# chenkovsky/aha

Measured on AMD Instinct MI355X. Metric: input GB/s scanned + M-hits/s, 100k-pattern AC over 1 GiB UTF-8 corpus, higher is better.
Workload: dtype u8

## Files before the change

### aha_amd/csrc/engine.cpp

```cpp
#include "handle.hpp"

#include <chrono>

namespace ahai {

constexpr size_t kLdsPerCU = 160 * 1024;
constexpr uint64_t kV2MaxRegionBytes = 48ull << 30;

bool skip_eligible(const aha_ac *ac) {
  const UnitImage &u = ac->unit;
  if (!u.ok || u.base_bits != 22 || u.unit_key || u.mark_bloom.empty()) return false;
  const char *eng = getenv("AHA_ENGINE");
  if (eng && strcmp(eng, "skip") != 0) return false;
  const char *hb = getenv("AHA_UNIT_HEADER_BESIDE");
  if (hb ? atoi(hb) != 0 : (!eng && (uint64_t)u.n_nfr * 5 >= u.n_states)) return false;
  const char *sk = getenv("AHA_SKIP");
  if (sk) return atoi(sk) != 0;
  return eng != nullptr;
}

bool pair_eligible(const aha_ac *ac) {
  const UnitImage &u = ac->unit;
  if (!u.ok || u.base_bits != 22 || u.unit_key || u.pair_tab.empty() || u.mark_bloom.empty() || u.deep_ends_max > kPairMaxDeepEnds ||
      ac->aut.max_key_len > 255)
// ... 297 lines not shown
  z[kSlabUsed] = direct ? 0 : n_slabs * 4;
  z[kEvCnt] = n_chunks * 4;
  z[kDocEvRank] = n_docs1 * 4;
  z[kEvBase] = n_chunks * 8;
  z[kBlkA] = z[kBlkB] = n_blk * 8;
  z[kCursor] = kCursorBytes;
  z[kEvAux] = z[kSortedAux] = chars ? ev_cap * 4 : 0;
  z[kLeadCnt] = z[kChunkDoc0] = (chars || pair) ? n_chunks * 4 : 0;
  z[kDocLeadRank] = chars ? n_docs1 * 4 : 0;
  z[kLeadBase] = chars ? n_chunks * 8 : 0;
  z[kEvRegions] = (unit && ac->unit_fused) ? 0 : n_reg * 8;
  z[kText] = 0;
  z[kChunkHits] = direct ? n_chunks * 4 : 0;
  z[kHitBase] = direct ? n_chunks * 8 : 0;
  z[kDocHitRank] = unit ? n_docs1 * 4 : 0;
  z[kEvGroups] = unit ? n_reg * 12 : 0;
  z[kEngineA] = filt ? ((N + 63) / 64 + 2) * 8 : (skip ? skip_bitmap_bytes(N) : (pair ? n_chunks * 4 : 0));
  z[kEngineB] = filt ? n_chunks * filter_chunk_rec_bytes() : (pair ? pair_cand_bytes(cand_cap) : 0);
  z[kEngineC] = pair ? pair_walk_bytes(cand_cap) : 0;
  z[kKeyVisits] = 0;
  return 0;
}

constexpr int32_t kNoRegions = 5;
static int32_t launch_v2(aha_ac *ac, Scratch *sc, MatchArgs &M1, const V2Plan &P, V2Args &M, bool prof, hipStream_t s) {
  const uint64_t N = M1.n_bytes;
  const bool counting = M1.count_only != 0, direct = P.direct, filt = P.filt, pair = P.pair, unit = P.unit, skip = P.skip;
  M = V2Args{};
  M.doc_off = M1.doc_off;
  M.n_docs = M1.n_docs;
  M.n_bytes = N;
  M.S = (uint32_t)P.S;
  M.n_chunks = P.n_chunks;
  M.lds_slots = ac->v2_lds_slots;
  M.chars = M1.chars;
  M.sep = M1.sep;
  memcpy(M.sep_block, M1.sep_block, sizeof(M.sep_block));
  M.out = M1.out;
  M.cap = M1.cap;
  M.doc_hit_off = M1.doc_hit_off;
  M.unit_bb = ac->unit.base_bits;
  M.direct = direct ? 1 : 0;
  M.dense_hits = P.dense ? 1 : 0;
  M.ev_stride = (uint32_t)P.stride;
  M.ev_cap = P.ev_cap;
  int32_t rc;
  for (int i = 0; i < kV2Count; i++) {
    if (!P.sizes[i]) continue;
    if ((rc = v2_reserve(sc, (V2Slot)i, P.sizes[i]))) return ((i == kEvRegions || i == kEvGroups) && P.mode != kSlabs) ? kNoRegions : rc;
  }
  if (M1.fold && !filt && (rc = stage_folded(ac, sc, M1, s))) return rc;
  const bool fold_loads = filt && M1.fold;
  auto at = [sc](V2Slot slot) { return sc->v2buf[slot].p; };
  M.text = M1.text;
  M.ev = (uint4 *)at(kEv);
  M.sorted_ev = (uint4 *)at(kSortedEv);
  M.sorted_cnt = (uint32_t *)at(kSortedCnt);
  M.slab_used = (uint32_t *)at(kSlabUsed);
  M.ev_cnt = (uint32_t *)at(kEvCnt);
  M.doc_ev_rank = (uint32_t *)at(kDocEvRank);
  M.ev_base = (uint64_t *)at(kEvBase);
  M.blk_a = (uint64_t *)at(kBlkA);
  M.blk_b = (uint64_t *)at(kBlkB);
  if (sc->cursor_buf != at(kCursor)) {
    sc->cursor_buf = at(kCursor);
    sc->cursor_dirty = true;
  }
  M.ev_aux = (uint32_t *)at(kEvAux);
  M.sorted_aux = (uint32_t *)at(kSortedAux);
  M.lead_cnt = (uint32_t *)at(kLeadCnt);
  M.chunk_doc0 = (uint32_t *)at(kChunkDoc0);
  M.doc_lead_rank = (uint32_t *)at(kDocLeadRank);
  M.lead_base = (uint64_t *)at(kLeadBase);
  M.evd = (uint2 *)at(kEvRegions);
  M.evg = (uint32_t *)at(kEvGroups);
  M.doc_hit_rank = (uint32_t *)at(kDocHitRank);
  M.chunk_hits = (uint32_t *)at(kChunkHits);
  M.hit_base = (uint64_t *)at(kHitBase);
  if ((rc = ensure_h_v2(ac, sc))) return rc;
  M.publish = (direct && M.doc_hit_off && sc->h_v2_dev) ? sc->h_v2_dev : nullptr;
  static const bool always_clear = getenv("AHA_CURSOR_MEMSET") != nullptr;
  if (sc->cursor_dirty || always_clear) {
    HIPCHK(ac, hipMemsetAsync(at(kCursor), 0, kCursorBytes, s));
    sc->cursor_phase = 0;
  }
  M.cursor = (unsigned long long *)at(kCursor) + 16 * sc->cursor_phase;
  M.totals = (uint64_t *)M.cursor + 2;
  M.clear_next = M.publish ? (unsigned long long *)at(kCursor) + 16 * (sc->cursor_phase ^ 1u) : nullptr;
  sc->cursor_dirty = true;

  if (M1.check_docs) launch_check_docs(M.doc_off, M.n_docs, N, nullptr, M.cursor + 1, s);
  if (M1.kc_visits) HIPCHK(ac, hipMemsetAsync(M1.kc_visits, 0, (size_t)ac->aut.n_keys * 8, s));
  if (prof) HIPCHK(ac, hipEventRecord(sc->ev[0], s));
  const uint64_t n_tiles = (M.n_chunks + kV2Threads - 1) / kV2Threads;
  DevAut post = ac->dev;
  if (pair) {
    post.end_info = ac->d_unit_end_info;
    post.compact = 1;
    pair_launch(ac->pdev, ac->udev, post, M, at(kEngineA), at(kEngineB), at(kEngineC), P.cand_cap, ac->v2_grid,
                prof ? (void *)sc->ev[2] : nullptr, s);
  } else if (unit) {
    post.end_info = ac->d_unit_end_info;
    post.compact = 1;
    if (skip) {
      skip_launch_mark(ac->sdev, M, at(kEngineA), ac->v2_grid, s);
      if (prof) HIPCHK(ac, hipEventRecord(sc->ev[2], s));
      skip_launch_traverse(ac->udev, M, at(kEngineA), (uint32_t)std::min<uint64_t>(ac->v2_grid, n_tiles), s);
    } else {
      unit_launch_traverse(ac->udev, M, (uint32_t)std::min<uint64_t>(ac->v2_grid, n_tiles), s);
    }
  } else if (filt) {
    unsigned long long *non_ascii = M1.chars ? M.cursor + 6 : nullptr;
    (fold_loads ? filter_launch_filter_fold : filter_launch_filter)(ac->fdev, M, at(kEngineA), at(kEngineB), non_ascii, ac->pf_cus, s);
    if (prof) HIPCHK(ac, hipEventRecord(sc->ev[2], s));
    (fold_loads ? filter_launch_walk_fold : filter_launch_walk)(ac->dev, M, at(kEngineA), at(kEngineB), non_ascii, ac->pf_cus, s);
  } else {
    v2_launch_traverse(ac->dev, M, (uint32_t)std::min<uint64_t>(ac->v2_grid, n_tiles), s);
  }
  if (prof) HIPCHK(ac, hipEventRecord(sc->ev[1], s));
  if (counting) {
    const unsigned long long *abortf = (const unsigned long long *)(M.cursor + 1);
    static const long count_blocks_env = getenv("AHA_COUNT_BLOCKS") ? atol(getenv("AHA_COUNT_BLOCKS")) : 0;
    const uint32_t count_blocks = count_blocks_env > 0 ? (uint32_t)count_blocks_env : 4u * ac->v2_grid;
    uint64_t *cdoc = nullptr;
    if (M1.cover_mask) {
      if (!(cdoc = (uint64_t *)cover_reserve(sc, kCovChunkDoc, (M.n_chunks + 1) * 8))) {
        tls_err = "hipMalloc failed for the scratch of a cover call";
        return AHA_E_HIP;
      }
      if (M1.cover_clear) cover_launch_clear(M1.cover_mask, (N + 31) / 32, abortf, 8u * ac->v2_grid, s);
    }
    if (unit && ac->unit_fused) {
      v2_launch_hit_scan(M, s);
      if (prof) HIPCHK(ac, hipEventRecord(sc->ev[3], s));
      if (M1.kc_visits) count_launch_visits(post, M, ac->d_unit_end, M1.kc_visits, count_blocks, s);
      if (cdoc) cover_launch_spans(post, M, ac->d_unit_end, cdoc, M1.cover_mask, M1.cover_bit0, count_blocks, s);
    } else {
      if (unit) unit_launch_regroup(post, M, s);
      v2_launch_count_post(post, M, s, unit || filt || pair);
      if (prof) HIPCHK(ac, hipEventRecord(sc->ev[3], s));
      if (M1.kc_visits) count_launch_visits(post, M, nullptr, M1.kc_visits, count_blocks, s);
      if (cdoc) cover_launch_spans(post, M, nullptr, cdoc, M1.cover_mask, M1.cover_bit0, count_blocks, s);
    }
    if (M1.kc_visits) count_launch_chain(ac->dev.key_ln, ac->aut.n_keys, M1.kc_visits, M1.kc_out, abortf, s);
    if (unit && ac->unit_fused)
      unit_launch_doc_offsets(M, s);
    else
      v2_launch_doc_offsets(post, M, s);
  } else if (direct) {
    if (unit && ac->unit_fused) {
      v2_launch_hit_scan(M, s);
      if (M.chars) v2_launch_lead_scan(M, s);
      if (prof) HIPCHK(ac, hipEventRecord(sc->ev[3], s));
      unit_launch_expand(M.chars ? ac->d_unit_end_chars : ac->d_unit_end, post, M, 2u * ac->v2_grid, s);
    } else {
      if (unit) unit_launch_regroup(post, M, s);
      v2_launch_direct_post(post, M, s, prof ? (void *)sc->ev[3] : nullptr, unit || filt || pair);
    }
  } else {
    v2_launch_chunk_scan(M, s);
    if (prof) HIPCHK(ac, hipEventRecord(sc->ev[2], s));
    v2_launch_sort(ac->dev, M, M.ev_cap, s);
    if (prof) HIPCHK(ac, hipEventRecord(sc->ev[3], s));
    v2_launch_expand(ac->dev, M, M.ev_cap, s);
  }
  if (prof) HIPCHK(ac, hipEventRecord(sc->ev[4], s));
  HIPCHK(ac, hipGetLastError());
  return AHA_OK;
}

static int32_t verdict_v2(aha_ac *ac, Scratch *sc, MatchArgs &M1, const V2Plan &P, const V2Args &M, bool prof, hipStream_t s,
                          uint64_t *n_hits) {
  const bool counting = M1.count_only != 0, direct = P.direct, filt = P.filt, pair = P.pair, unit = P.unit, skip = P.skip;
  [[maybe_unused]] const uint64_t N = M1.n_bytes;
  if (M.publish) {
  } else if (sc->h_v2_dev) {
    launch_publish_words((const unsigned long long *)M.cursor, sc->h_v2_dev, 5, s);
  } else {
    HIPCHK(ac, hipMemcpyAsync(sc->h_v2, M.cursor, 5 * 8, hipMemcpyDeviceToHost, s));
  }
  HIPCHK(ac, hipStreamSynchronize(s));
  if (M.clear_next) {
    sc->cursor_dirty = false;
    sc->cursor_phase ^= 1u;
  }
#ifdef AHA_EXPAND_CLK
  {
    unsigned long long w[16];
    (void)hipMemcpy(w, M.cursor, sizeof(w), hipMemcpyDeviceToHost);
    if (w[15])
      fprintf(stderr, "k2d_expand_dense, %llu sampled chunks, %.1f windows each; cycles per window: A %.0f  B2 %.0f  wait %.0f  fill %.0f  wall-clock ticks of 10 ns per chunk %.0f; clocks per chunk %.0f\n",
              w[15], (double)w[13] / w[15], (double)w[8] / w[13], (double)w[9] / w[13], (double)w[10] / w[13], (double)w[11] / w[13], (double)w[12] / w[15],
              (double)w[14] / w[15]);
    if (w[7]) fprintf(stderr, "  blocks sampled %llu: %.1f chunks each, %.0f clocks from the kernel's first instruction to its stores' acknowledgement\n", w[7], (double)w[6] / w[7], (double)w[5] / w[7]);
  }
#endif
#ifdef AHA_SK_STATS
  if (skip) {
    unsigned long long w[16];
    (void)hipMemcpy(w, M.cursor, sizeof(w), hipMemcpyDeviceToHost);
    fprintf(stderr, "ks_traverse: %llu lane-trips (%.4f per byte), %llu jumps, %llu fresh, %llu wave-trips (%.1f %% of the lane slots used)\n", w[8],
            (double)w[8] / (double)N, w[9], w[11], w[10], 100.0 * (double)w[8] / (64.0 * (double)w[10]));
  }
#endif
  if (sc->h_v2[1] >= 16) return bad_offsets(sc->h_v2[1] & 1);
  if (sc->h_v2[1] == 3 && pair) {
    if (!counting && !M1.neutral) ac->pair_off.fetch_add(1, std::memory_order_relaxed);
    M1.no_pair = 1;
  }
  if (sc->h_v2[1] == 3) return 3;
  M1.check_docs = 0;
  if (sc->h_v2[1] == 2) return 2;
  if (sc->h_v2[1]) return 1;
  *n_hits = sc->h_v2[2];
  if (prof) {
    aha_timing t{};
    t.engine = pair ? 7 : (skip ? 6 : (unit ? 4 : (filt ? 5 : 2)));
    t.chunk_bytes = M.S;
    t.n_kernels = 9;
    t.n_chunks = M.n_chunks;
    t.n_hits = *n_hits;
    const bool front = filt || skip || pair;
    if (direct)
      publish_event_timing(ac, sc, t, front ? 2 : 1, front ? 2 : -1, 1, 1, 3);
    else
      publish_event_timing(ac, sc, t, front ? 2 : 1, 1, 2, 2, 3);
  }
  return AHA_OK;
}

static int32_t match_v2(aha_ac *ac, Scratch *sc, MatchArgs &M1, hipStream_t s, uint64_t *n_hits, V2Mode mode) {
  for (;;) {
    V2Plan P;
    int32_t rc = plan_v2(ac, M1, mode, P);
    if (rc) return rc;
    if (P.want_pair && !P.direct) {
      M1.no_pair = 1;
      mode = P.mode;
      continue;
    }
    V2Args M;
    const bool prof = ac->profiling.load() && sc->ev_ready;
    rc = launch_v2(ac, sc, M1, P, M, prof, s);
    if (rc == kNoRegions) {
      if (M1.count_only) return 4;
      mode = kSlabs;
      continue;
    }
    if (rc) return rc;
    return verdict_v2(ac, sc, M1, P, M, prof, s, n_hits);
  }
}

int32_t ready_events(aha_ac *ac, Scratch *sc) {
  if (!ac->profiling.load() || sc->ev_ready) return AHA_OK;
  static const unsigned ev_flags = getenv("AHA_EVENT_FENCE") ? hipEventDefault : hipEventDisableSystemFence;
  for (auto &e : sc->ev) HIPCHK(ac, hipEventCreateWithFlags(&e, ev_flags));
  sc->ev_ready = true;
  return AHA_OK;
}

static int32_t check_docs_now(aha_ac *ac, Scratch *sc, const uint64_t *d_doc_offsets, uint64_t n_docs, uint64_t n_bytes,
                              hipStream_t s) {
  int32_t rc2;
  if ((rc2 = v2_reserve(sc, kCursor, kCursorBytes))) return rc2;
  if ((rc2 = ensure_h_v2(ac, sc))) return rc2;
  uint32_t *flag = (uint32_t *)sc->v2buf[kCursor].p + 64;
  HIPCHK(ac, hipMemsetAsync(flag, 0, 4, s));
  launch_check_docs(d_doc_offsets, n_docs, n_bytes, flag, nullptr, s);
  HIPCHK(ac, hipMemcpyAsync(sc->h_v2, flag, 4, hipMemcpyDeviceToHost, s));
  HIPCHK(ac, hipStreamSynchronize(s));
  const uint32_t bad = (uint32_t)sc->h_v2[0];
  return (bad & 3u) ? bad_offsets(bad & 1u) : AHA_OK;
}

int32_t device_match(aha_ac *ac, Scratch *sc, const uint8_t *d_corpus, const uint64_t *d_doc_offsets, uint64_t n_docs,
                     uint64_t n_bytes, const aha_match_params *params, aha_hit *d_out, uint64_t cap, uint64_t *d_doc_hit_offsets,
                     uint64_t *n_hits, void *stream, bool offsets_checked, const PackOut *pk, bool *packed, bool quiet, bool neutral) {
  if (!ac || !n_hits || !d_doc_offsets) return AHA_E_INVALID;
  if (ac->device < 0) return no_device();
  if (cap && !d_out) return AHA_E_INVALID;
  DeviceGuard g(ac->device);
  hipStream_t s = (hipStream_t)stream;
  MatchArgs M{};
  int longest = 0;
  int32_t rc = fill_params(ac, params, M, &longest);
  if (rc) return rc;
  if ((rc = ready_events(ac, sc))) return rc;
  if (quiet) M.no_filter = M.no_pair = 1;
  M.neutral = neutral ? 1 : 0;
  *n_hits = 0;
  auto check_now = [&]() { return check_docs_now(ac, sc, d_doc_offsets, n_docs, n_bytes, s); };
  auto fits = [&]() {
    if (*n_hits <= cap) return (int32_t)AHA_OK;
    tls_err = "output buffer too small";
    return (int32_t)AHA_E_CAPACITY;
  };
  const bool defer_check = !offsets_checked && ac->v2_ok && !longest && n_bytes != 0;
  if (!offsets_checked && !defer_check && (rc = check_now())) return rc;
  M.check_docs = defer_check ? 1 : 0;
  if (n_bytes == 0) {
    if (d_doc_hit_offsets)
      HIPCHK(ac, hipMemsetAsync(d_doc_hit_offsets, 0, (n_docs + 1) * sizeof(uint64_t), s));
    HIPCHK(ac, hipStreamSynchronize(s));
    return AHA_OK;
  }
  if (!d_corpus) return AHA_E_INVALID;
// ... 903 lines not shown
```

### aha_amd/csrc/image.hpp

```cpp
#pragma once
#include <cstdint>

#include "../../include/aha_hip.h"

namespace aha {

struct DevAut {
  const void *slots;
  const int32_t *end_key;
  const uint32_t *end_info;
  const uint2 *key_ln;
  const uint32_t *key_cnt;
  const uint32_t *key_kc;
  const uint32_t *key_info;
  const uint2 *chain;
  const uint2 *chain_chars;
  uint32_t root;
  uint32_t n_slots;
  uint32_t max_len;
  uint32_t compact;
  uint32_t s1_lo;
  uint32_t s2_lo;
  uint32_t s2_hi;
  const uint32_t *stale_bits;
  const uint32_t *term_bits;
};

struct MatchArgs {
  const uint8_t *text;
  const uint64_t *doc_off;
  uint64_t n_docs;
  uint64_t n_bytes;
  uint64_t n_chunks;
  uint32_t chunk;
  int32_t chars;
  int32_t sep;
  uint32_t sep_block[8];
  int32_t has_nul;
  int32_t no_filter;
  int32_t no_pair;
  int32_t check_docs;
  uint32_t *counts;
  uint32_t *leads;
  uint64_t *blk_hits;
  uint64_t *blk_leads;
  uint64_t *docg;
  uint64_t *totals;
  aha_hit *out;
  uint64_t cap;
  uint64_t *doc_hit_off;
  int32_t count_only;
  unsigned long long *kc_visits;
  unsigned long long *kc_hits;
  unsigned long long *kc_out;
  int32_t neutral;
  uint32_t *cover_mask;
  uint64_t cover_bit0;
  int32_t cover_clear;
  int32_t fold;
};

constexpr int kBlock = 256;

constexpr int kV2Threads = 1024;
constexpr int kV2Piece = 32;
constexpr uint32_t kV2Slab = 512;
constexpr uint32_t kV2MaxS = 32768;

struct V2Args {
  const uint8_t *text;
  const uint64_t *doc_off;
  uint64_t n_docs;
  uint64_t n_bytes;
  uint64_t n_chunks;
  uint32_t S;
  uint32_t lds_slots;
  int32_t chars;
  int32_t sep;
  uint32_t sep_block[8];
  uint4 *ev;
  uint32_t *ev_aux;
  uint64_t ev_cap;
  unsigned long long *cursor;
  uint32_t *slab_used;
  uint32_t *ev_cnt;
  uint32_t *lead_cnt;
  uint32_t *chunk_doc0;
  uint32_t *doc_ev_rank;
  uint32_t *doc_lead_rank;
  uint64_t *ev_base;
  uint64_t *lead_base;
  uint64_t *blk_a;
  uint64_t *blk_b;
  uint4 *sorted_ev;
  uint32_t *sorted_aux;
  uint32_t *sorted_cnt;
  uint64_t *totals;
  int32_t direct;
  int32_t dense_hits;
  uint32_t ev_stride;
  uint2 *evd;
  uint32_t *evg;
  uint32_t *doc_hit_rank;
  uint32_t unit_bb;
  uint32_t *chunk_hits;
  uint64_t *hit_base;
  aha_hit *out;
  uint64_t cap;
  uint64_t *doc_hit_off;
  unsigned long long *publish;
  unsigned long long *clear_next;
  uint32_t doc_from, doc_lanes16;
};

struct UnitDev {
  const uint2 *slots;
  const uint32_t *root;
  const uint32_t *tables;
  uint32_t n_slots;
  uint32_t big_lo;
  uint32_t n_low;
  uint32_t g0;
  uint32_t base_bits;
  uint32_t n_syms;
  uint32_t max_len;
  uint32_t hdr_beside;
};
size_t unit_lds_bytes(uint32_t n_syms);
int unit_prepare(uint32_t n_syms);
void unit_launch_traverse(const UnitDev &U, const V2Args &M, uint32_t grid, void *stream);
void unit_launch_regroup(const DevAut &A, const V2Args &M, void *stream);
void unit_launch_expand(const uint2 *uend, const DevAut &A, const V2Args &M, uint32_t workgroups, void *stream);
void v2_launch_hit_scan(const V2Args &M, void *stream);
void v2_launch_lead_scan(const V2Args &M, void *stream);

struct SkipDev {
  const uint32_t *bloom;
  uint32_t log2;
  uint32_t k1;
};
int skip_prepare(uint32_t n_syms, uint32_t log2_words);
size_t skip_bitmap_bytes(uint64_t n_bytes);
void skip_launch_mark(const SkipDev &K, const V2Args &M, void *bitmap, uint32_t grid, void *stream);
void skip_launch_traverse(const UnitDev &U, const V2Args &M, const void *bitmap, uint32_t grid, void *stream);

struct PairDev {
  const uint32_t *bloom;
  const uint4 *tab;
  const uint8_t *disp;
  uint32_t bloom_log2, k1, log2, groups;
};

int pair_prepare(uint32_t n_syms, uint32_t bloom_log2, uint32_t groups);
uint32_t pair_tile_bytes();
size_t pair_cand_bytes(uint64_t cap);
size_t pair_walk_bytes(uint64_t cap);
void pair_launch(const PairDev &P, const UnitDev &U, const DevAut &A, const V2Args &M, void *tile_dn, void *cand, void *wres,
                 uint64_t cand_cap, uint32_t grid, void *mid_event, void *stream);

constexpr uint32_t kFilterMul = 0x9E3779B1u;
constexpr uint32_t kFilterLog2 = 14;
struct FilterDev {
  const uint32_t *bloom;
  uint32_t d;
  uint32_t log2;
};
bool filter_image_in_lds(uint32_t n_slots, uint32_t chunk_bytes, bool chars = false);
int filter_prepare();
size_t filter_chunk_rec_bytes();
void filter_launch_filter(const FilterDev &F, const V2Args &M, void *bitmap, void *chunk_rec, unsigned long long *non_ascii,
                          uint32_t cus, void *stream);
void filter_launch_walk(const DevAut &A, const V2Args &M, const void *bitmap, const void *chunk_rec, const unsigned long long *non_ascii,
                        uint32_t cus, void *stream);

void filter_launch_filter_fold(const FilterDev &F, const V2Args &M, void *bitmap, void *chunk_rec, unsigned long long *non_ascii,
                               uint32_t cus, void *stream);
void filter_launch_walk_fold(const DevAut &A, const V2Args &M, const void *bitmap, const void *chunk_rec,
                             const unsigned long long *non_ascii, uint32_t cus, void *stream);
void fold_launch_copy(const uint8_t *src, uint8_t *dst, uint64_t n_bytes, uint32_t max_blocks, void *stream);

size_t v2_lds_bytes(uint32_t lds_slots, bool compact);
int v2_prepare(bool compact, size_t lds_bytes);
void v2_launch_traverse(const DevAut &A, const V2Args &M, uint32_t grid, void *stream);
void v2_launch_chunk_scan(const V2Args &M, void *stream);
void v2_launch_sort(const DevAut &A, const V2Args &M, uint64_t n_records, void *stream);
void v2_launch_expand(const DevAut &A, const V2Args &M, uint64_t n_events, void *stream);
void v2_launch_direct_post(const DevAut &A, const V2Args &M, void *stream, void *ev_mid, bool counted = false);
void v2_launch_count_post(const DevAut &A, const V2Args &M, void *stream, bool counted);
void v2_launch_doc_offsets(const DevAut &A, const V2Args &M, void *stream);
void unit_launch_doc_offsets(const V2Args &M, void *stream);
void count_launch_visits(const DevAut &A, const V2Args &M, const uint2 *uend, unsigned long long *visits, uint32_t max_blocks,
                         void *stream);
void count_launch_chain(const uint2 *key_ln, uint32_t n_keys, const unsigned long long *visits, unsigned long long *out,
                        const unsigned long long *abortf, void *stream);

void cover_launch_clear(uint32_t *words, uint64_t n_words, const unsigned long long *abortf, uint32_t max_blocks, void *stream);
void cover_launch_spans(const DevAut &A, const V2Args &M, const uint2 *uend, uint64_t *cdoc, uint32_t *mask, uint64_t bit0,
                        uint32_t max_blocks, void *stream);
void cover_launch_redact(const uint8_t *src, uint8_t *dst, const uint32_t *mask, uint64_t n_bytes, uint8_t fill, uint32_t max_blocks,
                         void *stream);
void cover_launch_doc_covered(const uint32_t *mask, const uint64_t *doc_off, uint64_t n_docs, uint64_t *doc_covered,
                              uint32_t max_blocks, void *stream);
void cover_launch_total(const uint32_t *mask, uint64_t n_words, uint64_t *total, uint32_t max_blocks, void *stream);

struct DcItem {
  uint64_t begin;
  uint32_t *out;
  uint32_t n;
  uint32_t doc;
};
constexpr uint32_t kDcSortMax = 4096;
constexpr uint32_t kDcRangeKeys = 8192;
constexpr uint32_t kDcSliceHits = 1u << 16;
void doccount_launch_sort(const DcItem *items, uint32_t n_items, const void *hits, uint32_t *n_pairs, void *stream);
void doccount_launch_range(const DcItem *items, uint32_t n_items, const void *hits, uint32_t n_keys, uint32_t range_keys,
                           uint32_t *n_pairs, void *stream);
void doccount_launch_add(const DcItem *slices, uint32_t n_slices, const void *hits, uint32_t *rows, uint32_t n_keys,
                         uint32_t max_blocks, void *stream);
void doccount_launch_compact(const DcItem *docs, uint32_t n_rows, uint32_t *rows, uint32_t n_keys, uint32_t *n_pairs, void *stream);
void doccount_launch_compact64(const DcItem *doc, unsigned long long *row, uint32_t n_keys, uint32_t *n_pairs, void *stream);
void doccount_launch_gather(const uint64_t *pair_off, const uint32_t *const *src, uint64_t n_docs, uint64_t n, void *out,
                            void *stream);

uint64_t select_rank_blocks(uint64_t n_bytes);
void select_launch_longest(const void *hits, uint64_t n_hits, const uint64_t *hit_off, const uint64_t *rel, uint64_t nd, uint64_t nb,
                           uint64_t *L, uint32_t max_blocks, void *stream);
void select_launch_marks(const uint64_t *L, uint64_t nb, const uint64_t *rel, uint64_t nd, uint32_t *cover, uint32_t *doc_start,
                         uint32_t max_blocks, void *stream);
void select_launch_walk(const uint64_t *L, uint64_t nb, const uint32_t *cover, const uint32_t *doc_start, uint32_t *select,
                        uint32_t max_blocks, void *stream);
void select_launch_rank(const uint32_t *select, uint64_t nb, uint64_t *blk, uint32_t max_blocks, void *stream);
void select_launch_rank_docs(const uint32_t *select, const uint64_t *blk, const uint64_t *rel, uint64_t nd, uint64_t base,
                             uint64_t *out, uint32_t max_blocks, void *stream);
void select_launch_emit(const uint32_t *select, uint64_t nb, const uint64_t *blk, const uint64_t *L, const uint64_t *rel, uint64_t nd,
                        void *out, uint32_t max_blocks, void *stream);

struct RepEntry {
  uint64_t off;
  uint32_t len;
  uint32_t keep;
};
constexpr uint32_t kRpScanBlock = 256;
inline uint64_t replace_scan_blocks(uint64_t n) { return (n + kRpScanBlock - 1) / kRpScanBlock; }
void replace_launch_delta(const void *sel, uint64_t n, const uint64_t *dso, const uint64_t *doc_off, uint64_t n_docs,
                          const RepEntry *ent, uint32_t n_keys, uint64_t *start, int64_t *shift, uint32_t max_blocks, void *stream);
void replace_launch_scan(int64_t *shift, uint64_t n, int64_t *sums, uint32_t max_blocks, void *stream);
void replace_launch_doc_offsets(const uint64_t *doc_off, const uint64_t *dso, const int64_t *shift, uint64_t n_docs,
                                uint64_t *doc_out, uint32_t max_blocks, void *stream);
void replace_launch_copy(const uint8_t *text, const void *sel, const uint64_t *start, const int64_t *shift, uint64_t n,
                         const RepEntry *ent, uint32_t n_keys, const uint8_t *blob, uint8_t *out, uint64_t total,
                         uint32_t max_blocks, void *stream);

void launch_hits_pack(const int32_t *hits, uint64_t n, int32_t *pairs, void *stream);
void launch_hits_unpack(const DevAut &A, const int32_t *pairs, uint64_t n, int chars, int32_t *hits, void *stream);
struct StreamFmt {
  uint32_t step_bits;
  uint32_t len_bits;
};
void launch_hits_pack4(const int32_t *hits, uint64_t n, uint32_t *stream_words, unsigned long long *n_words, StreamFmt F,
                       void *stream);
void launch_hits_unpack4(const DevAut &A, const uint32_t *stream_words, uint64_t n, int chars, int32_t *hits, StreamFmt F,
                         void *stream);
constexpr uint32_t kMaxSegs = 64;
void launch_hits_unpack4_segs(const DevAut &A, const uint32_t *land, const uint64_t *word_off, const uint64_t *n_hits,
                              const uint64_t *out_off, uint32_t n_segs, int chars, int32_t *hits, StreamFmt F, void *stream);

void launch_publish_words(const unsigned long long *src, unsigned long long *host_dst, int n, void *stream);
void launch_check_docs(const uint64_t *doc_off, uint64_t n_docs, uint64_t n_bytes, uint32_t *flag, unsigned long long *abort_word,
                       void *stream);

void launch_count(const DevAut &A, const MatchArgs &M, void *stream);
void launch_scan_blocks(const MatchArgs &M, uint64_t n_blocks, void *stream);
void launch_count_doc_offsets(const MatchArgs &M, void *stream);
void launch_docg(const MatchArgs &M, void *stream);
void launch_write(const DevAut &A, const MatchArgs &M, void *stream);
void launch_has_nul(const uint8_t *text, uint64_t n, uint64_t *flag, void *stream);
void launch_longest(const DevAut &A, const MatchArgs &M, int mode, bool write, void *stream);

}
```

### aha_amd/csrc/scan_unit.hip

```cpp
#include <hip/hip_runtime.h>

#include "automaton.hpp"
#include "devcommon.hpp"
#include "image.hpp"
#include "unit.hpp"

namespace aha {

namespace {

constexpr int kUPiece = 16;
constexpr int kUWin = 3 * kUPiece;
constexpr int kURow = kUWin + 4;
constexpr int kUWave = 64 * kURow;

__device__ __forceinline__ uint4 load16(const uint8_t *text, int64_t g, int64_t N) {
  uint4 v = make_uint4(0, 0, 0, 0);
  if (g >= 0 && g + 16 <= N) {
    v = *reinterpret_cast<const uint4 *>(text + g);
  } else if (g >= 0 && g < N) {
    uint32_t w0 = 0, w1 = 0, w2 = 0, w3 = 0;
#pragma unroll 1
    for (int j = 0; j < 16 && g + j < N; j++) {
      const uint32_t b = (uint32_t)text[g + j] << ((j & 3) * 8);
// ... 263 lines not shown
                d[1] = ry;
                d[2] = rz;
              }
            }
            wfill = (wfill + kp) & 63u;
            seq += ev ? 1u : 0u;
            hits += evc;
          }
        }
        if (all_left || !wany(rel < lim)) break;
      }
      if (need) pos = pb - 4 + rel;
    }
    {
      const uint32_t *q = reinterpret_cast<const uint32_t *>(smem + (wbo + __umul24((uint32_t)lane, 12u)));
      const v3u r = {q[0], q[1], q[2]};
      if ((uint32_t)lane < wfill && wout + (uint32_t)lane < wcap) *reinterpret_cast<v3u *>(wreg + (size_t)(wout + lane) * 3) = r;
    }
    if (live) {
      M.ev_cnt[chunk] = seq;
      if (seq > ev_stride) M.cursor[1] = 2ull;
      if (CHARS) M.lead_cnt[chunk] = lead_total;
      M.chunk_hits[chunk] = hits;
      if (e == N) {
        while (dn <= D) {
          M.doc_ev_rank[dn] = seq;
          M.doc_hit_rank[dn] = hits;
          if (CHARS) M.doc_lead_rank[dn] = lead_total;
          dn++;
        }
      }
    }
  }
}

constexpr int kRgThreads = 256, kRgPer = 4, kRgBlock = kRgThreads * kRgPer, kRgSubs = kRgBlock / 64;
__global__ __launch_bounds__(kRgThreads) void ku_regroup(DevAut A, V2Args M) {
  __shared__ uint2 s_sorted[kRgBlock];
  __shared__ uint8_t s_lane[kRgBlock];
  __shared__ uint32_t s_cnt[kRgSubs][64], s_part[kRgThreads / 64][64];
  __shared__ uint32_t s_start[64], s_tot[64], s_run[64], s_hits[64];
  if (M.cursor[1]) return;
  const int lane = threadIdx.x & 63, wv = threadIdx.x >> 6;
  const uint64_t n_groups = (M.n_chunks + 63) / 64;
  const uint32_t stride = M.ev_stride;
  const uint32_t bb = M.unit_bb, bmask = (1u << bb) - 1u;
  for (uint64_t g = blockIdx.x; g < n_groups; g += gridDim.x) {
    __syncthreads();
    if (wv == 0) {
      s_run[lane] = 0;
      s_hits[lane] = 0;
    }
    const uint64_t c = g * 64 + lane;
    uint32_t total = c < M.n_chunks ? min(M.ev_cnt[c], stride) : 0u;
#pragma unroll
    for (int d = 32; d >= 1; d >>= 1) total += __shfl_xor(total, d, 64);
    const uint32_t *src = M.evg + g * 64 * stride * 3;
    uint2 *dst = M.evd + g * 64 * stride;
    uint2 nxt[kRgPer];
    uint32_t xn[kRgPer];
#pragma unroll
    for (int q = 0; q < kRgPer; q++) {
      const uint32_t i = q * kRgThreads + threadIdx.x;
      nxt[q] = i < total ? make_uint2(src[(size_t)i * 3], src[(size_t)i * 3 + 1]) : make_uint2(0, 0);
    }
#pragma unroll
    for (int q = 0; q < kRgPer; q++) xn[q] = (uint32_t)(q * kRgThreads) + threadIdx.x < total ? A.end_info[nxt[q].x & bmask] : 0u;
    for (uint32_t i0 = 0; i0 < total; i0 += kRgBlock) {
      uint2 rec[kRgPer];
      uint32_t x[kRgPer], rank[kRgPer], l[kRgPer];
      bool live[kRgPer];
#pragma unroll
      for (int q = 0; q < kRgPer; q++) {
        const uint32_t i = i0 + q * kRgThreads + threadIdx.x;
        live[q] = i < total;
        rec[q] = nxt[q];
        x[q] = xn[q];
        nxt[q] = i + kRgBlock < total ? make_uint2(src[(size_t)(i + kRgBlock) * 3], src[(size_t)(i + kRgBlock) * 3 + 1])
                                      : make_uint2(0, 0);
      }
#pragma unroll
      for (int q = 0; q < kRgPer; q++) {
        l[q] = (rec[q].x >> bb) & 63u;
        uint64_t same = __ballot(live[q]), mine = same;
#pragma unroll
        for (int b = 0; b < 6; b++) {
          const uint64_t bal = __ballot(live[q] & ((l[q] >> b) & 1u) != 0u);
          same &= ((l[q] >> b) & 1u) ? bal : ~bal;
          mine &= ((lane >> b) & 1) ? bal : ~bal;
        }
        rank[q] = __popcll(same & ((1ull << lane) - 1ull));
        s_cnt[q * (kRgThreads / 64) + wv][lane] = __popcll(mine);
      }
      __syncthreads();
      {
        uint32_t acc = 0;
#pragma unroll
        for (int r = 0; r < kRgSubs / (kRgThreads / 64); r++) {
          const uint32_t v = s_cnt[wv * (kRgSubs / (kRgThreads / 64)) + r][lane];
          s_cnt[wv * (kRgSubs / (kRgThreads / 64)) + r][lane] = acc;
          acc += v;
        }
        s_part[wv][lane] = acc;
      }
      __syncthreads();
      if (wv == 0) {
        uint32_t acc = 0;
#pragma unroll
        for (int w2 = 0; w2 < kRgThreads / 64; w2++) {
          const uint32_t v = s_part[w2][lane];
          s_part[w2][lane] = acc;
          acc += v;
        }
        s_tot[lane] = acc;
        s_start[lane] = wave_incl_scan(acc) - acc;
      }
      __syncthreads();
#pragma unroll
      for (int q = 0; q < kRgPer; q++) {
        if (live[q]) {
          const uint32_t sb = q * (kRgThreads / 64) + wv;
          const uint32_t p = s_start[l[q]] + s_part[sb / (kRgSubs / (kRgThreads / 64))][l[q]] + s_cnt[sb][l[q]] + rank[q];
          uint32_t cnt = x[q] >> 24;
          if (cnt == 255u) cnt = A.key_cnt[A.chain ? A.chain[x[q] & 0xFFFFFFu].y : (x[q] & 0xFFFFFFu)];
          s_sorted[p] = make_uint2(x[q], rec[q].y);
          s_lane[p] = (uint8_t)l[q];
          if (cnt) atomicAdd(&s_hits[l[q]], cnt);
        }
      }
      __syncthreads();
#pragma unroll
      for (int q = 0; q < kRgPer; q++)
        xn[q] = i0 + kRgBlock + (uint32_t)(q * kRgThreads) + threadIdx.x < total ? A.end_info[nxt[q].x & bmask] : 0u;
#pragma unroll
      for (int q = 0; q < kRgPer; q++) asm volatile("" : "+v"(xn[q]));
      const uint32_t nb = min(total - i0, (uint32_t)kRgBlock);
#pragma unroll
      for (int q = 0; q < kRgPer; q++) {
        const uint32_t p = q * kRgThreads + threadIdx.x;
        if (p < nb) {
          const uint32_t lp = s_lane[p];
          const uint32_t at = s_run[lp] + (p - s_start[lp]);
          if (at < stride) dst[(uint64_t)lp * stride + at] = s_sorted[p];
        }
      }
      __syncthreads();
      if (wv == 0) s_run[lane] += s_tot[lane];
    }
    __syncthreads();
    if (wv == 0 && c < M.n_chunks) M.chunk_hits[c] = s_hits[lane];
  }
}

constexpr int kXgThreads = 1024, kXgPer = 1, kXgBlock = kXgThreads * kXgPer, kXgStage = 1536;
constexpr int kXgCacheBits = 11;
template <bool CHARS>
__global__ __launch_bounds__(kXgThreads) void ku_expand_groups(const uint2 *uend, DevAut A, V2Args M) {
  __shared__ uint32_t s_hs[kXgStage], s_he[kXgStage], s_hk[kXgStage];
  __shared__ uint8_t s_hl[kXgStage];
  __shared__ uint32_t s_tot[2][64], s_start[64], s_run[64], s_all;
  __shared__ uint64_t s_base[64];
  __shared__ uint32_t s_adj[64];
  __shared__ unsigned long long s_cache[1 << kXgCacheBits];
  if (M.cursor[1]) return;
  const int lane = threadIdx.x & 63, wv = threadIdx.x >> 6;
  const uint64_t n_groups = (M.n_chunks + 63) / 64;
  const uint32_t stride = M.ev_stride;
  const uint32_t bb = M.unit_bb, bmask = (1u << bb) - 1u;
  for (uint32_t i = threadIdx.x; i < (1u << kXgCacheBits); i += kXgThreads) s_cache[i] = 0ull;
  for (uint64_t g = blockIdx.x; g < n_groups; g += gridDim.x) {
    __syncthreads();
    const uint64_t c = g * 64 + lane;
    if (wv == 0) {
      if (CHARS && c < M.n_chunks) s_adj[lane] = M.lead_cnt[c];
      s_base[lane] = c < M.n_chunks ? M.hit_base[c] : 0ull;
      s_run[lane] = 0;
      s_tot[0][lane] = 0;
    }
    uint32_t total = c < M.n_chunks ? min(M.ev_cnt[c], stride) : 0u;
#pragma unroll
    for (int d = 32; d >= 1; d >>= 1) total += __shfl_xor(total, d, 64);
    const uint32_t *src = M.evg + g * 64 * stride * 3;
    typedef uint32_t v3u __attribute__((ext_vector_type(3)));
    v3u nxt[kXgPer];
#pragma unroll
    for (int q = 0; q < kXgPer; q++) {
      const uint32_t i = q * kXgThreads + threadIdx.x;
      nxt[q] = i < total ? __builtin_nontemporal_load(reinterpret_cast<const v3u *>(src + (size_t)i * 3)) : v3u{0, 0, 0};
    }
    __syncthreads();
    uint32_t par = 0;
    for (uint32_t i0 = 0; i0 < total; i0 += kXgBlock, par ^= 1u) {
      v3u rec[kXgPer];
      uint2 ue[kXgPer];
      bool live[kXgPer], keep[kXgPer];
      uint32_t cs[kXgPer];
#pragma unroll
      for (int q = 0; q < kXgPer; q++) {
        const uint32_t i = i0 + q * kXgThreads + threadIdx.x;
        live[q] = i < total;
        rec[q] = nxt[q];
        nxt[q] = i + kXgBlock < total ? __builtin_nontemporal_load(reinterpret_cast<const v3u *>(src + (size_t)(i + kXgBlock) * 3)) : v3u{0, 0, 0};
        const uint32_t b = rec[q].x & bmask, n = u_rec_n(rec[q].x, rec[q].z, bb);
        cs[q] = (b * 0x9E3779B1u) >> (32 - kXgCacheBits);
        const unsigned long long ce = s_cache[cs[q]];
        const bool cached = live[q] & n == 1u & (uint32_t)ce == b + 1u;
        ue[q] = make_uint2((uint32_t)(ce >> 32), 0u);
        if (live[q] && !cached) ue[q] = uend[b];
        keep[q] = live[q] & !cached & n == 1u;
        if (live[q]) atomicAdd(&s_tot[par][(rec[q].x >> bb) & 63u], n);
      }
      __syncthreads();
      if (wv == 0) {
        const uint32_t t = s_tot[par][lane];
        const uint32_t incl = wave_incl_scan(t);
        s_start[lane] = incl - t;
        if (lane == 63) s_all = incl;
        s_tot[par ^ 1u][lane] = 0;
      }
      __syncthreads();
      const uint32_t T = s_all;
#pragma unroll
      for (int q = 0; q < kXgPer; q++)
        if (keep[q] && (ue[q].y >> 24) == 0u)
          atomicExch(&s_cache[cs[q]], (unsigned long long)ue[q].x << 32 | ((rec[q].x & bmask) + 1u));
      for (uint32_t w0 = 0; w0 < T; w0 += kXgStage) {
#pragma unroll
        for (int q = 0; q < kXgPer; q++) {
          if (live[q]) {
            const uint32_t l = (rec[q].x >> bb) & 63u, n = u_rec_n(rec[q].x, rec[q].z, bb);
            const uint32_t pos = s_start[l] + (u_rec_before(rec[q].z) - s_run[l]);
            const uint32_t end = CHARS ? (rec[q].y >> 1) + ((rec[q].y & 1u) ? 0u : s_adj[l]) : rec[q].y, co = ue[q].y & 0xFFFFFFu;
            uint32_t len = (ue[q].x >> 24) | (ue[q].y >> 24) << 8, key = ue[q].x & 0xFFFFFFu;
            for (uint32_t k = 0;;) {
              const uint32_t j = pos + k - w0;
              if (j < (uint32_t)kXgStage) {
                s_hs[j] = end - len;
                s_he[j] = end;
                s_hk[j] = key;
                s_hl[j] = (uint8_t)l;
              }
              if (++k >= n) break;
              const uint2 ce = (CHARS ? A.chain_chars : A.chain)[co + k];
              len = ce.x;
              key = ce.y;
            }
          }
        }
        __syncthreads();
        const uint32_t nh = min(T - w0, (uint32_t)kXgStage);
        for (uint32_t j = threadIdx.x; j < nh; j += kXgThreads) {
          const uint32_t l = s_hl[j];
          const uint64_t idx = s_base[l] + s_run[l] + (w0 + j - s_start[l]);
          if (idx < M.cap) {
            aha_hit hit;
            hit.start = (int32_t)s_hs[j];
            hit.end = (int32_t)s_he[j];
            hit.value = (int32_t)s_hk[j];
            M.out[idx] = hit;
          }
        }
        __syncthreads();
      }
      if (wv == 0) s_run[lane] += s_tot[par][lane];
    }
  }
}

__global__ __launch_bounds__(256) void ku_chunk_adj(V2Args M) {
  if (M.cursor[1]) return;
  const uint64_t c = (uint64_t)blockIdx.x * 256 + threadIdx.x;
  if (c >= M.n_chunks) return;
  const uint32_t d0 = M.chunk_doc0[c];
  const uint64_t dchunk = M.doc_off[d0] / M.S;
  M.lead_cnt[c] = (uint32_t)(M.lead_base[c] - (M.lead_base[dchunk] + M.doc_lead_rank[d0]));
}

__global__ __launch_bounds__(256) void ku_doc_offsets(V2Args M) {
  if (M.publish && blockIdx.x == 0 && threadIdx.x < 5) M.publish[threadIdx.x] = M.cursor[threadIdx.x];
  if (M.clear_next && blockIdx.x == 0 && threadIdx.x < 16) M.clear_next[threadIdx.x] = 0ull;
  if (M.cursor[1] || !M.doc_hit_off) return;
  const uint64_t d = (uint64_t)blockIdx.x * 256 + threadIdx.x;
  if (d > M.n_docs) return;
  const uint64_t q = M.doc_off[d];
  M.doc_hit_off[d] = q < M.n_bytes ? M.hit_base[q / M.S] + M.doc_hit_rank[d] : M.totals[0];
}

}

size_t unit_lds_bytes(uint32_t n_syms) { return u_lds(n_syms); }

int unit_prepare(uint32_t n_syms) {
  const int lds = (int)unit_lds_bytes(n_syms);
  int e = 0;
#define AHA_PREP_KU(C, B, H) \
  if (!e) e = (int)hipFuncSetAttribute((const void *)ku_traverse<C, B, H>, hipFuncAttributeMaxDynamicSharedMemorySize, lds);
  AHA_PREP_KU(false, 22, false) AHA_PREP_KU(true, 22, false) AHA_PREP_KU(false, 23, false) AHA_PREP_KU(true, 23, false)
  AHA_PREP_KU(false, 22, true) AHA_PREP_KU(true, 22, true) AHA_PREP_KU(false, 23, true) AHA_PREP_KU(true, 23, true)
#undef AHA_PREP_KU
  return e;
}

void unit_launch_traverse(const UnitDev &U, const V2Args &M, uint32_t grid, void *stream) {
  const size_t lds = unit_lds_bytes(U.n_syms);
#define AHA_LAUNCH_KU(C, B, H) hipLaunchKernelGGL((ku_traverse<C, B, H>), dim3(grid), dim3(kV2Threads), lds, (hipStream_t)stream, U, M)
#define AHA_LAUNCH_KU2(C, B) \
  do {                       \
    if (U.hdr_beside)        \
      AHA_LAUNCH_KU(C, B, true);  \
    else                     \
      AHA_LAUNCH_KU(C, B, false); \
  } while (0)
  if (U.base_bits == 23) {
    if (M.chars) AHA_LAUNCH_KU2(true, 23); else AHA_LAUNCH_KU2(false, 23);
  } else {
    if (M.chars) AHA_LAUNCH_KU2(true, 22); else AHA_LAUNCH_KU2(false, 22);
  }
#undef AHA_LAUNCH_KU2
#undef AHA_LAUNCH_KU
}

void unit_launch_doc_offsets(const V2Args &M, void *stream) {
  if (M.doc_hit_off)
    hipLaunchKernelGGL(ku_doc_offsets, dim3((uint32_t)((M.n_docs + 1 + 255) / 256)), dim3(256), 0, (hipStream_t)stream, M);
}

void unit_launch_regroup(const DevAut &A, const V2Args &M, void *stream) {
  const uint64_t n_groups = (M.n_chunks + 63) / 64;
  hipLaunchKernelGGL(ku_regroup, dim3((uint32_t)std::min<uint64_t>(n_groups, 1u << 16)), dim3(kRgThreads), 0,
                     (hipStream_t)stream, A, M);
}

void unit_launch_expand(const uint2 *uend, const DevAut &A, const V2Args &M, uint32_t workgroups, void *stream) {
  const uint64_t n_groups = (M.n_chunks + 63) / 64;
  const dim3 grid((uint32_t)std::max<uint64_t>(1, std::min<uint64_t>(n_groups, workgroups)));
  if (M.chars) {
    hipLaunchKernelGGL(ku_chunk_adj, dim3((uint32_t)((M.n_chunks + 255) / 256)), dim3(256), 0, (hipStream_t)stream, M);
    hipLaunchKernelGGL(ku_expand_groups<true>, grid, dim3(kXgThreads), 0, (hipStream_t)stream, uend, A, M);
  } else {
    hipLaunchKernelGGL(ku_expand_groups<false>, grid, dim3(kXgThreads), 0, (hipStream_t)stream, uend, A, M);
  }
  if (M.doc_hit_off)
    hipLaunchKernelGGL(ku_doc_offsets, dim3((uint32_t)((M.n_docs + 1 + 255) / 256)), dim3(256), 0, (hipStream_t)stream, M);
}

}
```

Before: 444.6.

## Restructure hit expansion into output-windowed LDS staging with coalesced vector stores

```diff
diff --git a/aha_amd/csrc/engine.cpp b/aha_amd/csrc/engine.cpp
--- a/aha_amd/csrc/engine.cpp
+++ b/aha_amd/csrc/engine.cpp
@@ -473,7 +473,7 @@
       v2_launch_hit_scan(M, s);
       if (M.chars) v2_launch_lead_scan(M, s);
       if (prof) HIPCHK(ac, hipEventRecord(sc->ev[3], s));
-      unit_launch_expand(M.chars ? ac->d_unit_end_chars : ac->d_unit_end, post, M, 2u * ac->v2_grid, s);
+      unit_launch_expand(M.chars ? ac->d_unit_end_chars : ac->d_unit_end, post, M, ac->v2_grid, s);
     } else {
       if (unit) unit_launch_regroup(post, M, s);
       v2_launch_direct_post(post, M, s, prof ? (void *)sc->ev[3] : nullptr, unit || filt || pair);
diff --git a/aha_amd/csrc/image.hpp b/aha_amd/csrc/image.hpp
--- a/aha_amd/csrc/image.hpp
+++ b/aha_amd/csrc/image.hpp
@@ -130,7 +130,7 @@
 int unit_prepare(uint32_t n_syms);
 void unit_launch_traverse(const UnitDev &U, const V2Args &M, uint32_t grid, void *stream);
 void unit_launch_regroup(const DevAut &A, const V2Args &M, void *stream);
-void unit_launch_expand(const uint2 *uend, const DevAut &A, const V2Args &M, uint32_t workgroups, void *stream);
+void unit_launch_expand(const uint2 *uend, const DevAut &A, const V2Args &M, uint32_t cus, void *stream);
 void v2_launch_hit_scan(const V2Args &M, void *stream);
 void v2_launch_lead_scan(const V2Args &M, void *stream);
 
diff --git a/aha_amd/csrc/scan_unit.hip b/aha_amd/csrc/scan_unit.hip
--- a/aha_amd/csrc/scan_unit.hip
+++ b/aha_amd/csrc/scan_unit.hip
@@ -439,117 +439,119 @@
   }
 }
 
-constexpr int kXgThreads = 1024, kXgPer = 1, kXgBlock = kXgThreads * kXgPer, kXgStage = 1536;
+#ifndef AHA_XG_PER
+#define AHA_XG_PER 4
+#endif
+constexpr int kXgThreads = 1024, kXgPer = AHA_XG_PER, kXgBlock = kXgThreads * kXgPer;
 constexpr int kXgCacheBits = 11;
+#ifndef AHA_XG_WINDOW
+#define AHA_XG_WINDOW 11264
+#define AHA_XG_PER_CU 1
+#endif
+constexpr uint32_t kXgWindow = AHA_XG_WINDOW;
+constexpr uint32_t kXgPerCU = AHA_XG_PER_CU;
+constexpr uint32_t kXgLdsBase = 8u << kXgCacheBits, kXgLdsAdj = kXgLdsBase + 65u * 8u;
+constexpr uint32_t kXgLdsStage = (kXgLdsAdj + 64u * 4u + 15u) & ~15u;
+constexpr uint32_t kXgLds = kXgLdsStage + kXgWindow * 12u + 16u;
+static_assert(kXgLds * kXgPerCU <= 160u * 1024u, "the expansion's workgroups do not fit a CU's LDS");
 template <bool CHARS>
-__global__ __launch_bounds__(kXgThreads) void ku_expand_groups(const uint2 *uend, DevAut A, V2Args M) {
-  __shared__ uint32_t s_hs[kXgStage], s_he[kXgStage], s_hk[kXgStage];
-  __shared__ uint8_t s_hl[kXgStage];
-  __shared__ uint32_t s_tot[2][64], s_start[64], s_run[64], s_all;
-  __shared__ uint64_t s_base[64];
-  __shared__ uint32_t s_adj[64];
-  __shared__ unsigned long long s_cache[1 << kXgCacheBits];
+__global__ __launch_bounds__(kXgThreads, kXgThreads / 256 * kXgPerCU) void ku_expand_groups(const uint2 *uend, DevAut A, V2Args M) {
+  extern __shared__ __attribute__((aligned(16))) uint8_t smem[];
+  unsigned long long *s_cache = reinterpret_cast<unsigned long long *>(smem);
+  uint64_t *s_base = reinterpret_cast<uint64_t *>(smem + kXgLdsBase);
+  uint32_t *s_adj = reinterpret_cast<uint32_t *>(smem + kXgLdsAdj);
+  uint32_t *s_stage = reinterpret_cast<uint32_t *>(smem + kXgLdsStage);
   if (M.cursor[1]) return;
   const int lane = threadIdx.x & 63, wv = threadIdx.x >> 6;
   const uint64_t n_groups = (M.n_chunks + 63) / 64;
   const uint32_t stride = M.ev_stride;
   const uint32_t bb = M.unit_bb, bmask = (1u << bb) - 1u;
+  const uint64_t cap = M.cap;
   for (uint32_t i = threadIdx.x; i < (1u << kXgCacheBits); i += kXgThreads) s_cache[i] = 0ull;
+  typedef uint32_t v3u __attribute__((ext_vector_type(3)));
+  uint64_t nbase = 0, nend = 0;
+  uint32_t nev = 0, nadj = 0;
+  auto fetch_group = [&](uint64_t g) {
+    const uint64_t c = g * 64 + lane, c1 = g * 64 + 64;
+    const bool in = c < M.n_chunks;
+    nbase = in ? M.hit_base[c] : M.totals[0];
+    nend = c1 < M.n_chunks ? M.hit_base[c1] : M.totals[0];
+    nev = in ? min(M.ev_cnt[c], stride) : 0u;
+    if (CHARS) nadj = in ? M.lead_cnt[c] : 0u;
+  };
+  if (blockIdx.x < n_groups) fetch_group(blockIdx.x);
   for (uint64_t g = blockIdx.x; g < n_groups; g += gridDim.x) {
     __syncthreads();
-    const uint64_t c = g * 64 + lane;
     if (wv == 0) {
-      if (CHARS && c < M.n_chunks) s_adj[lane] = M.lead_cnt[c];
-      s_base[lane] = c < M.n_chunks ? M.hit_base[c] : 0ull;
-      s_run[lane] = 0;
-      s_tot[0][lane] = 0;
-    }
-    uint32_t total = c < M.n_chunks ? min(M.ev_cnt[c], stride) : 0u;
+      s_base[lane] = nbase;
+      if (lane == 0) s_base[64] = nend;
+      if (CHARS) s_adj[lane] = nadj;
+    }
+    uint32_t total = nev;
 #pragma unroll
     for (int d = 32; d >= 1; d >>= 1) total += __shfl_xor(total, d, 64);
+    const uint64_t span0 = min(__shfl(nbase, 0, 64), cap), span1 = min(nend, cap);
+    if (g + gridDim.x < n_groups) fetch_group(g + gridDim.x);
     const uint32_t *src = M.evg + g * 64 * stride * 3;
-    typedef uint32_t v3u __attribute__((ext_vector_type(3)));
-    v3u nxt[kXgPer];
-#pragma unroll
-    for (int q = 0; q < kXgPer; q++) {
-      const uint32_t i = q * kXgThreads + threadIdx.x;
-      nxt[q] = i < total ? __builtin_nontemporal_load(reinterpret_cast<const v3u *>(src + (size_t)i * 3)) : v3u{0, 0, 0};
-    }
     __syncthreads();
-    uint32_t par = 0;
-    for (uint32_t i0 = 0; i0 < total; i0 += kXgBlock, par ^= 1u) {
-      v3u rec[kXgPer];
-      uint2 ue[kXgPer];
-      bool live[kXgPer], keep[kXgPer];
-      uint32_t cs[kXgPer];
+    for (uint64_t w0 = span0; w0 < span1; w0 += kXgWindow) {
+      const uint32_t wl = (uint32_t)min<uint64_t>(span1 - w0, kXgWindow);
+      uint32_t *gp = reinterpret_cast<uint32_t *>(M.out) + w0 * 3;
+      const uint32_t sd = (uint32_t)(reinterpret_cast<uintptr_t>(gp) >> 2) & 3u;
+      uint32_t *st = s_stage + sd;
+      v3u nxt[kXgPer];
 #pragma unroll
       for (int q = 0; q < kXgPer; q++) {
-        const uint32_t i = i0 + q * kXgThreads + threadIdx.x;
-        live[q] = i < total;
-        rec[q] = nxt[q];
-        nxt[q] = i + kXgBlock < total ? __builtin_nontemporal_load(reinterpret_cast<const v3u *>(src + (size_t)(i + kXgBlock) * 3)) : v3u{0, 0, 0};
-        const uint32_t b = rec[q].x & bmask, n = u_rec_n(rec[q].x, rec[q].z, bb);
-        cs[q] = (b * 0x9E3779B1u) >> (32 - kXgCacheBits);
-        const unsigned long long ce = s_cache[cs[q]];
-        const bool cached = live[q] & n == 1u & (uint32_t)ce == b + 1u;
-        ue[q] = make_uint2((uint32_t)(ce >> 32), 0u);
-        if (live[q] && !cached) ue[q] = uend[b];
-        keep[q] = live[q] & !cached & n == 1u;
-        if (live[q]) atomicAdd(&s_tot[par][(rec[q].x >> bb) & 63u], n);
-      }
-      __syncthreads();
-      if (wv == 0) {
-        const uint32_t t = s_tot[par][lane];
-        const uint32_t incl = wave_incl_scan(t);
-        s_start[lane] = incl - t;
-        if (lane == 63) s_all = incl;
-        s_tot[par ^ 1u][lane] = 0;
-      }
-      __syncthreads();
-      const uint32_t T = s_all;
-#pragma unroll
-      for (int q = 0; q < kXgPer; q++)
-        if (keep[q] && (ue[q].y >> 24) == 0u)
-          atomicExch(&s_cache[cs[q]], (unsigned long long)ue[q].x << 32 | ((rec[q].x & bmask) + 1u));
-      for (uint32_t w0 = 0; w0 < T; w0 += kXgStage) {
+        const uint32_t i = q * kXgThreads + threadIdx.x;
+        nxt[q] = i < total ? __builtin_nontemporal_load(reinterpret_cast<const v3u *>(src + (size_t)i * 3)) : v3u{0, 0, 0};
+      }
+      for (uint32_t i0 = 0; i0 < total; i0 += kXgBlock) {
+        v3u rec[kXgPer];
 #pragma unroll
         for (int q = 0; q < kXgPer; q++) {
-          if (live[q]) {
-            const uint32_t l = (rec[q].x >> bb) & 63u, n = u_rec_n(rec[q].x, rec[q].z, bb);
-            const uint32_t pos = s_start[l] + (u_rec_before(rec[q].z) - s_run[l]);
-            const uint32_t end = CHARS ? (rec[q].y >> 1) + ((rec[q].y & 1u) ? 0u : s_adj[l]) : rec[q].y, co = ue[q].y & 0xFFFFFFu;
-            uint32_t len = (ue[q].x >> 24) | (ue[q].y >> 24) << 8, key = ue[q].x & 0xFFFFFFu;
-            for (uint32_t k = 0;;) {
-              const uint32_t j = pos + k - w0;
-              if (j < (uint32_t)kXgStage) {
-                s_hs[j] = end - len;
-                s_he[j] = end;
-                s_hk[j] = key;
-                s_hl[j] = (uint8_t)l;
+          const uint32_t i = i0 + kXgBlock + q * kXgThreads + threadIdx.x;
+          rec[q] = nxt[q];
+          nxt[q] = i < total ? __builtin_nontemporal_load(reinterpret_cast<const v3u *>(src + (size_t)i * 3)) : v3u{0, 0, 0};
+        }
+#pragma unroll
+        for (int q = 0; q < kXgPer; q++) {
+          const bool live = i0 + q * kXgThreads + threadIdx.x < total;
+          const uint32_t l = (rec[q].x >> bb) & 63u, n = u_rec_n(rec[q].x, rec[q].z, bb);
+          const int64_t rel = (int64_t)(s_base[l] + u_rec_before(rec[q].z) - w0);
+          if (live && rel < (int64_t)wl && rel + (int64_t)n > 0) {
+            const uint32_t b = rec[q].x & bmask, cs = (b * 0x9E3779B1u) >> (32 - kXgCacheBits);
+            const unsigned long long ce = __hip_atomic_load(&s_cache[cs], __ATOMIC_RELAXED, __HIP_MEMORY_SCOPE_WORKGROUP);
+            uint2 ue = make_uint2((uint32_t)(ce >> 32), 0u);
+            if (!(n == 1u && (uint32_t)ce == b + 1u)) {
+              ue = uend[b];
+              if (n == 1u && (ue.y >> 24) == 0u)
+                __hip_atomic_store(&s_cache[cs], (unsigned long long)ue.x << 32 | (b + 1u), __ATOMIC_RELAXED, __HIP_MEMORY_SCOPE_WORKGROUP);
+            }
+            const uint32_t end = CHARS ? (rec[q].y >> 1) + ((rec[q].y & 1u) ? 0u : s_adj[l]) : rec[q].y, co = ue.y & 0xFFFFFFu;
+            uint32_t len = (ue.x >> 24) | (ue.y >> 24) << 8, key = ue.x & 0xFFFFFFu;
+            int32_t j = (int32_t)rel;
+            for (uint32_t k = 0;; j++) {
+              if ((uint32_t)j < wl) {
+                st[3 * j] = end - len;
+                st[3 * j + 1] = end;
+                st[3 * j + 2] = key;
               }
               if (++k >= n) break;
-              const uint2 ce = (CHARS ? A.chain_chars : A.chain)[co + k];
-              len = ce.x;
-              key = ce.y;
+              const uint2 cn = (CHARS ? A.chain_chars : A.chain)[co + k];
+              len = cn.x;
+              key = cn.y;
             }
           }
         }
-        __syncthreads();
-        const uint32_t nh = min(T - w0, (uint32_t)kXgStage);
-        for (uint32_t j = threadIdx.x; j < nh; j += kXgThreads) {
-          const uint32_t l = s_hl[j];
-          const uint64_t idx = s_base[l] + s_run[l] + (w0 + j - s_start[l]);
-          if (idx < M.cap) {
-            aha_hit hit;
-            hit.start = (int32_t)s_hs[j];
-            hit.end = (int32_t)s_he[j];
-            hit.value = (int32_t)s_hk[j];
-            M.out[idx] = hit;
-          }
-        }
-        __syncthreads();
-      }
-      if (wv == 0) s_run[lane] += s_tot[par][lane];
+      }
+      __syncthreads();
+      const uint32_t nd = wl * 3u, head = min(nd, (4u - sd) & 3u), nq = (nd - head) >> 2, tail = (nd - head) & 3u;
+      if (threadIdx.x < head) gp[threadIdx.x] = st[threadIdx.x];
+      const uint4 *sq = reinterpret_cast<const uint4 *>(st + head);
+      uint4 *gq = reinterpret_cast<uint4 *>(gp + head);
+      for (uint32_t p = threadIdx.x; p < nq; p += kXgThreads) gq[p] = sq[p];
+      if (threadIdx.x >= 64u && threadIdx.x - 64u < tail) gp[head + 4u * nq + (threadIdx.x - 64u)] = st[head + 4u * nq + (threadIdx.x - 64u)];
+      if (w0 + kXgWindow < span1) __syncthreads();
     }
   }
 }
@@ -585,6 +587,8 @@
   AHA_PREP_KU(false, 22, false) AHA_PREP_KU(true, 22, false) AHA_PREP_KU(false, 23, false) AHA_PREP_KU(true, 23, false)
   AHA_PREP_KU(false, 22, true) AHA_PREP_KU(true, 22, true) AHA_PREP_KU(false, 23, true) AHA_PREP_KU(true, 23, true)
 #undef AHA_PREP_KU
+  if (!e) e = (int)hipFuncSetAttribute((const void *)ku_expand_groups<false>, hipFuncAttributeMaxDynamicSharedMemorySize, (int)kXgLds);
+  if (!e) e = (int)hipFuncSetAttribute((const void *)ku_expand_groups<true>, hipFuncAttributeMaxDynamicSharedMemorySize, (int)kXgLds);
   return e;
 }
 
@@ -618,14 +622,14 @@
                      (hipStream_t)stream, A, M);
 }
 
-void unit_launch_expand(const uint2 *uend, const DevAut &A, const V2Args &M, uint32_t workgroups, void *stream) {
+void unit_launch_expand(const uint2 *uend, const DevAut &A, const V2Args &M, uint32_t cus, void *stream) {
   const uint64_t n_groups = (M.n_chunks + 63) / 64;
-  const dim3 grid((uint32_t)std::max<uint64_t>(1, std::min<uint64_t>(n_groups, workgroups)));
+  const dim3 grid((uint32_t)std::max<uint64_t>(1, std::min<uint64_t>(n_groups, (uint64_t)kXgPerCU * cus)));
   if (M.chars) {
     hipLaunchKernelGGL(ku_chunk_adj, dim3((uint32_t)((M.n_chunks + 255) / 256)), dim3(256), 0, (hipStream_t)stream, M);
-    hipLaunchKernelGGL(ku_expand_groups<true>, grid, dim3(kXgThreads), 0, (hipStream_t)stream, uend, A, M);
+    hipLaunchKernelGGL(ku_expand_groups<true>, grid, dim3(kXgThreads), kXgLds, (hipStream_t)stream, uend, A, M);
   } else {
-    hipLaunchKernelGGL(ku_expand_groups<false>, grid, dim3(kXgThreads), 0, (hipStream_t)stream, uend, A, M);
+    hipLaunchKernelGGL(ku_expand_groups<false>, grid, dim3(kXgThreads), kXgLds, (hipStream_t)stream, uend, A, M);
   }
   if (M.doc_hit_off)
     hipLaunchKernelGGL(ku_doc_offsets, dim3((uint32_t)((M.n_docs + 1 + 255) / 256)), dim3(256), 0, (hipStream_t)stream, M);
```

Result: no change. 443.3 (-0.3%).
